# aniketntnu/WordDiffusion

Measured on AMD Instinct MI355X. Metric: denoised 64x256 word images/sec (1000-step DDPM), whole job, higher is better.
Workload: dtype bf16x3; 1 GPU; BASELINE configs[1]: batch 64 per GPU of 64x256 crops = [64,4,8,32] latents, 1000-step DDPM (999 executed steps), base unet.py UNetModel (320 ch, mult (1,1), 4 heads, 339 writers), random-init synthetic weights; variant=base, batch_per_gpu=64, noise_steps=1000, executed_steps_per_image=999, precision=split-bf16 MFMA x3, fp32 accumulate (<=1e-4 of the fp32 reference), output_finite=True

## Files before the change

### worddiffusion_amd/csrc/wd_common.h

```cpp
#pragma once
#include <hip/hip_runtime.h>
#include <stdint.h>

#include "../../include/wdiff_hip.h"

#define WD_CLS_GEMM 0
#define WD_CLS_GNSTATS 1
#define WD_CLS_GNAPPLY 2
#define WD_CLS_LN 3
#define WD_CLS_ATTN 4
#define WD_CLS_OTHER 5
#define WD_CLS_GEMM_OTHER 6
#define WD_CLS_GEMM_REDUCE 7
#define WD_CLS_GEMM_2CU 8
#define WD_CLS_GEMM_WDIRECT 9
#define WD_CLS_FF 10
#define WD_CLS_DW 11
#define WD_CLS_GEMM_Q 12

extern "C" int wd_prof_is_on();
void wd_prof_begin(int cls, hipStream_t s, double flops);
void wd_prof_end(hipStream_t s);

struct WdLaunchScope {
    hipStream_t s;
    bool on;
    WdLaunchScope(int cls, hipStream_t st, double flops = 0.0) : s(st), on(wd_prof_is_on() != 0) {
        if (on) wd_prof_begin(cls, s, flops);
    }
    ~WdLaunchScope() {
        if (on) wd_prof_end(s);
    }
};

static inline int wd_check_launch() {
    hipError_t e = hipGetLastError();
    return e == hipSuccess ? WD_OK : WD_ELAUNCH;
}

__device__ __forceinline__ uint32_t wd_f2bf_bits(float x) {
    uint32_t u = __float_as_uint(x);
    return (u + 0x7FFFu + ((u >> 16) & 1u)) >> 16;
}
__device__ __forceinline__ float wd_bf_bits2f(uint32_t b) { return __uint_as_float(b << 16); }

typedef __attribute__((ext_vector_type(2))) float wd_f32x2;
typedef __attribute__((ext_vector_type(2))) __bf16 wd_bf16x2;
__device__ __forceinline__ uint32_t wd_pack_bf16x2(float a, float b) {
    const wd_f32x2 v = {a, b};
    return __builtin_bit_cast(uint32_t, __builtin_convertvector(v, wd_bf16x2));
}

__device__ __forceinline__ void wd_split1(float x, uint32_t& hi, uint32_t& lo) {
    hi = wd_pack_bf16x2(x, 0.f) & 0xffffu;
    lo = wd_pack_bf16x2(x - __uint_as_float(hi << 16), 0.f) & 0xffffu;
}

__device__ __forceinline__ void wd_split4(const float4 v, uint2& hi, uint2& lo) {
    const uint32_t h01 = wd_pack_bf16x2(v.x, v.y), h23 = wd_pack_bf16x2(v.z, v.w);
    hi = make_uint2(h01, h23);
    lo = make_uint2(wd_pack_bf16x2(v.x - __uint_as_float(h01 << 16), v.y - __uint_as_float(h01 & 0xffff0000u)),
                    wd_pack_bf16x2(v.z - __uint_as_float(h23 << 16), v.w - __uint_as_float(h23 & 0xffff0000u)));
}

__device__ __forceinline__ float wd_silu(float x) { return __fdividef(x, 1.0f + __expf(-x)); }
__device__ __forceinline__ float wd_erf(float x) {
    const float ax = fabsf(x);
    const float t = __fdividef(1.0f, 1.0f + 0.3275911f * ax);
    const float poly = t * (0.254829592f + t * (-0.284496736f + t * (1.421413741f + t * (-1.453152027f + t * 1.061405429f))));
    const float r = 1.0f - poly * __expf(-ax * ax);
    return copysignf(r, x);
}
__device__ __forceinline__ float wd_gelu_erf(float x) { return 0.5f * x * (1.0f + wd_erf(x * 0.70710678118654752440f)); }

template <int CTRL>
__device__ __forceinline__ float wd_dpp(float v) {
    return __int_as_float(__builtin_amdgcn_update_dpp(0, __float_as_int(v), CTRL, 0xf, 0xf, true));
}
__device__ __forceinline__ float wd_row16_sum(float v) {
    v += wd_dpp<0xB1>(v);
    v += wd_dpp<0x4E>(v);
    v += wd_dpp<0x124>(v);
    v += wd_dpp<0x128>(v);
    return v;
}
__device__ __forceinline__ float wd_wave_sum(float v) {
    v += wd_dpp<0xB1>(v);
    v += wd_dpp<0x4E>(v);
    v += wd_dpp<0x124>(v);
    v += wd_dpp<0x128>(v);
    const float r0 = __int_as_float(__builtin_amdgcn_readlane(__float_as_int(v), 0));
    const float r1 = __int_as_float(__builtin_amdgcn_readlane(__float_as_int(v), 16));
    const float r2 = __int_as_float(__builtin_amdgcn_readlane(__float_as_int(v), 32));
    const float r3 = __int_as_float(__builtin_amdgcn_readlane(__float_as_int(v), 48));
    return (r0 + r1) + (r2 + r3);
}
__device__ __forceinline__ float wd_wave_max(float v) {
    v = fmaxf(v, wd_dpp<0xB1>(v));
    v = fmaxf(v, wd_dpp<0x4E>(v));
    v = fmaxf(v, wd_dpp<0x124>(v));
    v = fmaxf(v, wd_dpp<0x128>(v));
    const float r0 = __int_as_float(__builtin_amdgcn_readlane(__float_as_int(v), 0));
    const float r1 = __int_as_float(__builtin_amdgcn_readlane(__float_as_int(v), 16));
    const float r2 = __int_as_float(__builtin_amdgcn_readlane(__float_as_int(v), 32));
    const float r3 = __int_as_float(__builtin_amdgcn_readlane(__float_as_int(v), 48));
    return fmaxf(fmaxf(r0, r1), fmaxf(r2, r3));
}
```

### worddiffusion_amd/csrc/wd_ff.hip

```cpp
#include "wd_gemm_epi.h"

namespace {

constexpr int FNT = 512;
constexpr int FBM = 64;
constexpr int FC = 320;
constexpr int FCH = 128;
constexpr int FRING = 6;
constexpr int F_MAX_INNER = 2048;
constexpr int FGRP = 30;
constexpr uint32_t F_OOB = 0x80000000u;

typedef __attribute__((ext_vector_type(4))) unsigned f_u32x4;

__device__ __forceinline__ int f_lds_off(int row, int ch) { return row * 128 + ((ch ^ ((row >> 1) & 7)) << 4); }

__host__ __device__ __forceinline__ wd_gemm_args ff_epi_args(const wd_ff_args& a, const bool proj, const bool fold) {
    wd_gemm_args e = {};
    e.m = a.m;
    e.n = FC;
    e.hw_out = a.hw_out > 0 ? a.hw_out : 1;
    e.act = WD_ACT_NONE;
    e.out_f32 = a.out_f32;
    e.out_ld = a.out_ld;
    e.out_hi = a.out_hi;
    e.out_lo = a.out_lo;
    e.out_pl_ld = a.out_pl_ld;
    e.ksplit = 1;
    e.stat_part = a.stat_part;
    e.stat_cpg = a.stat_cpg;
    e.bias = !proj ? a.b2 : fold ? a.b32 : a.b3;
    e.resid = proj ? a.resid3 : a.resid;
    e.resid_ld = proj ? a.resid3_ld : a.resid_ld;
    e.dbg = a.dbg;
    return e;
}

__device__ __forceinline__ void ff_epilogue(const wd_gemm_args& e, float* ep, const int m0, const int tid) {
    if ((e.dbg & WD_EPI_BATCH_BIT) && wd_epilogue_batch_ok(e, FBM, FC)) wd_epilogue_rows<FBM, FC, FNT>(e, ep, m0, 0, tid);
    else wd_epilogue_from_image<FBM, FC, FNT>(e, ep, m0, 0, tid);
}

template <int NPASS, bool PROJ, bool FRONT, bool FOLD>
__global__ void __launch_bounds__(FNT, 1) wd_ff_kernel(const wd_ff_args a) {
#if defined(__HIP_DEVICE_COMPILE__)
    static_assert(!FRONT || (NPASS == 3 && PROJ), "the transformer front needs split-bf16 operands and the proj_out tail");
    static_assert(!FOLD || (NPASS == 3 && PROJ), "the folded tail is the proj_out tail in split-bf16");
    constexpr int NPL = (NPASS == 1) ? 1 : 2;
    constexpr int SLAB = 2 * FBM * 128;
    constexpr int A_BYTES = 5 * SLAB;
    constexpr int H_BYTES = 2 * SLAB;
    extern __shared__ __attribute__((aligned(16))) char smem[];
    char* s_a = smem;
    char* s_h = smem + A_BYTES;
    float* s_b1 = reinterpret_cast<float*>(smem + A_BYTES + 2 * H_BYTES);

    const int m0 = blockIdx.x * FBM;
    const int tid = threadIdx.x;
    const int lane = tid & 63;
    const int wave = __builtin_amdgcn_readfirstlane(tid >> 6);
    const int kh = wave >> 2, cg = wave & 3;
    const int l15 = lane & 15, lq = lane >> 4;
    const int nchunk = a.inner / FCH;

    auto make_srd = [](const wd_bf16* p) {
        return __builtin_amdgcn_make_buffer_rsrc(const_cast<wd_bf16*>(p), 0, 0x7FFFFFF0, 0x00020000);
    };
    const __amdgpu_buffer_rsrc_t srd1_hi = make_srd(a.w1_hi), srd1_lo = make_srd(a.w1_lo ? a.w1_lo : a.w1_hi);
    const __amdgpu_buffer_rsrc_t srd2_hi = make_srd(FOLD ? a.w32_hi : a.w2_hi),
                                 srd2_lo = make_srd(FOLD ? a.w32_lo : a.w2_lo ? a.w2_lo : a.w2_hi);
    const __amdgpu_buffer_rsrc_t srd3_hi = make_srd(PROJ ? a.w3_hi : a.w2_hi), srd3_lo = make_srd(PROJ ? (a.w3_lo ? a.w3_lo : a.w3_hi) : a.w2_hi);
    const uint32_t lane16 = lane * 16;
    const int nct1 = (2 * a.inner) >> 4;

    bf16x8 ring[FRING][NPL];
    auto issue = [&](const int slot, const int g, const int j) {
        const bool live = j < nchunk;
        const uint32_t vo = live ? lane16 : F_OOB;
        if (PROJ && !FOLD && g < FRING) {
            const uint32_t so3 = (uint32_t)(((2 * (g / 5) + kh) * (FC / 16) + 5 * cg + g % 5) * 1024);
            const uint32_t so1 = (uint32_t)(((g >> 1) * nct1 + 2 * (j * 8 + wave) + (g & 1)) * 1024);
            const uint32_t so = live ? so1 : so3;
#pragma unroll
            for (int p = 0; p < NPL; ++p) {
                const __amdgpu_buffer_rsrc_t srd = live ? (p ? srd1_lo : srd1_hi) : (p ? srd3_lo : srd3_hi);
                ring[slot][p] = __builtin_bit_cast(bf16x8, __builtin_amdgcn_raw_buffer_load_b128(srd, lane16, so, 0));
            }
        } else if (g < 20) {
            const uint32_t so = (uint32_t)(((g >> 1) * nct1 + 2 * (j * 8 + wave) + (g & 1)) * 1024);
#pragma unroll
            for (int p = 0; p < NPL; ++p)
                ring[slot][p] = __builtin_bit_cast(bf16x8, __builtin_amdgcn_raw_buffer_load_b128(p ? srd1_lo : srd1_hi, vo, live ? so : 0u, 0));
        } else {
            const int q = (g - 20) / 5, t = (g - 20) % 5;
            const uint32_t so = (uint32_t)(((4 * j + 2 * kh + q) * (FC / 16) + 5 * cg + t) * 1024);
#pragma unroll
            for (int p = 0; p < NPL; ++p)
                ring[slot][p] = __builtin_bit_cast(bf16x8, __builtin_amdgcn_raw_buffer_load_b128(p ? srd2_lo : srd2_hi, vo, live ? so : 0u, 0));
        }
    };
    f32x4 acc2[4][5];
    bf16x8 xa[4][NPL];
    auto read_frags = [&](const char* slab_base, const int half) {
        const int ch = half * 4 + lq;
#pragma unroll
        for (int i = 0; i < 4; ++i) {
            const int ao = f_lds_off(i * 16 + l15, ch);
#pragma unroll
            for (int p = 0; p < NPL; ++p) xa[i][p] = *reinterpret_cast<const bf16x8*>(slab_base + p * (FBM * 128) + ao);
        }
    };
    auto mfma12 = [&](f32x4 (&acc)[4], const bf16x8 (&w)[NPL]) {
#pragma unroll
        for (int i = 0; i < 4; ++i) {
            if (NPL == 2) {
                acc[i] = __builtin_amdgcn_mfma_f32_16x16x32_bf16(xa[i][NPL - 1], w[0], acc[i], 0, 0, 0);
                acc[i] = __builtin_amdgcn_mfma_f32_16x16x32_bf16(xa[i][0], w[NPL - 1], acc[i], 0, 0, 0);
            }
            acc[i] = __builtin_amdgcn_mfma_f32_16x16x32_bf16(xa[i][0], w[0], acc[i], 0, 0, 0);
        }
    };
    constexpr int LDE = FC + 4;
    float* ep = reinterpret_cast<float*>(smem);
    auto ksum_to_image = [&]() {
        for (int hh = 0; hh < 2; ++hh) {
            if (kh == hh) {
#pragma unroll
                for (int i = 0; i < 4; ++i)
#pragma unroll
                    for (int t = 0; t < 5; ++t)
#pragma unroll
                        for (int r = 0; r < 4; ++r) {
                            float* pe = ep + (i * 16 + 4 * lq + r) * LDE + cg * 80 + t * 16 + l15;
                            *pe = (hh == 0) ? acc2[i][t][r] : *pe + acc2[i][t][r];
                        }
            }
            __syncthreads();
        }
    };

    auto issue_w3 = [&](const int slot, const int g) {
        const uint32_t so = (uint32_t)(((2 * (g / 5) + kh) * (FC / 16) + 5 * cg + g % 5) * 1024);
#pragma unroll
        for (int p = 0; p < NPL; ++p)
            ring[slot][p] = __builtin_bit_cast(bf16x8, __builtin_amdgcn_raw_buffer_load_b128(p ? srd3_lo : srd3_hi, lane16, so, 0));
    };
    auto fold_product = [&](const int q0, const int q1, const char* slabs) {
        if (q0 == 0) {
#pragma unroll
            for (int i = 0; i < 4; ++i)
#pragma unroll
                for (int t = 0; t < 5; ++t)
#pragma unroll
                    for (int r = 0; r < 4; ++r) acc2[i][t][r] = 0.0f;
        }
#pragma unroll
        for (int g = 0; g < 25; ++g) {
            const int q = g / 5, t = g % 5;
            if (q < q0 || q >= q1) continue;
            if (t == 0) read_frags(slabs + (q - q0) * SLAB, kh);
            {
                f32x4 col[4] = {acc2[0][t], acc2[1][t], acc2[2][t], acc2[3][t]};
                mfma12(col, ring[(g + 5) % FRING]);
#pragma unroll
                for (int i = 0; i < 4; ++i) acc2[i][t] = col[i];
            }
            if (g + FRING < 25) issue_w3((g + 5) % FRING, g + FRING);
            else issue((g + 5) % FRING, g + FRING - 25, 0);
            __builtin_amdgcn_sched_barrier(0);
        }
    };

    if constexpr (FRONT) {
        constexpr int SP = 65, PP = 72, KS32 = FC / 32;
        const int b = m0 / a.hw;
        const int HJ = a.heads * a.L;
        char* fr = s_h + 4096;
        float* s_aff = reinterpret_cast<float*>(fr);
        float* sS = reinterpret_cast<float*>(fr);
        wd_bf16* sP = reinterpret_cast<wd_bf16*>(fr + FBM * SP * 4);
        float* s_vec = reinterpret_cast<float*>(s_h + (FOLD ? 49152 : 40960));
        const float* s_pib = s_vec;
        const float* s_ln2g = s_vec + FC, * s_ln2b = s_vec + 2 * FC, * s_ln3g = s_vec + 3 * FC, * s_ln3b = s_vec + 4 * FC;
        const float* s_xba = s_vec + 5 * FC, * s_xbb = s_vec + 6 * FC;
        const int arow = tid >> 3, ach = tid & 7;
        float4 xv[5][2];
        {
            const float* xrow = a.x_in + (long)(m0 + arow) * a.x_in_ld + ach * 8;
#pragma unroll
            for (int sl = 0; sl < 5; ++sl) {
                xv[sl][0] = *reinterpret_cast<const float4*>(xrow + sl * 64);
                xv[sl][1] = *reinterpret_cast<const float4*>(xrow + sl * 64 + 4);
            }
        }
        const __amdgpu_buffer_rsrc_t srdp_hi = make_srd(a.pi_hi), srdp_lo = make_srd(a.pi_lo);
        auto issue_pi = [&](const int slot, const int g) {
            const uint32_t so = (uint32_t)(((2 * (g / 5) + kh) * (FC / 16) + 5 * cg + g % 5) * 1024);
#pragma unroll
            for (int p = 0; p < NPL; ++p)
                ring[slot][p] = __builtin_bit_cast(bf16x8, __builtin_amdgcn_raw_buffer_load_b128(p ? srdp_lo : srdp_hi, lane16, so, 0));
        };
#pragma unroll
        for (int g = 0; g < FRING; ++g) issue_pi(g, g);
        const int sv = wave < 7 ? wave : 6;
        const float* vsrc = sv == 0 ? a.pi_b : sv == 1 ? a.ln2_gamma : sv == 2 ? a.ln2_beta : sv == 3 ? a.ln3_gamma : sv == 4 ? a.ln3_beta
                            : sv == 5 ? a.xb_a : a.xb_b;
        const float4 vst0 = *reinterpret_cast<const float4*>(vsrc + lane * 4);
        const float4 vst1 = *reinterpret_cast<const float4*>(vsrc + (64 + l15) * 4);
        constexpr int NB1 = 2 * F_MAX_INNER / FNT;
        float b1v[NB1];
        {
            const __amdgpu_buffer_rsrc_t sb1 = __builtin_amdgcn_make_buffer_rsrc(const_cast<float*>(a.b1), 0, a.b1 ? 2 * a.inner * 4 : 0, 0x00020000);
#pragma unroll
            for (int k = 0; k < NB1; ++k)
                b1v[k] = __builtin_bit_cast(float, __builtin_amdgcn_raw_buffer_load_b32(sb1, (uint32_t)(tid + k * FNT) * 4u, 0, 0));
        }
        __builtin_amdgcn_sched_barrier(0);
        for (int e = tid; e < FBM * PP; e += FNT) reinterpret_cast<uint32_t*>(sP)[e] = 0u;
        {
            const int ngp = FC / a.gn_pcpg, ratio = a.gn_cpg / a.gn_pcpg;
            for (int c = tid; c < FC; c += FNT) {
                const int g = c / a.gn_cpg;
                const float gam = a.gn_gamma[c], bet = a.gn_beta[c];
                double su = 0.0, sq = 0.0;
                const int nterm = ratio * a.gn_nchunk;
                int k = 0, ck = 0;
                for (int t0 = 0; t0 < nterm; t0 += 8) {
                    const int k0 = k, ck0 = ck;
                    double2 pv[8];
#pragma unroll
                    for (int u = 0; u < 8; ++u) {
                        const bool live = t0 + u < nterm;
                        const int kk = live ? k : k0, cc = live ? ck : ck0;
                        pv[u] = *reinterpret_cast<const double2*>(a.gn_part + (((long)b * a.gn_nchunk + cc) * ngp + g * ratio + kk) * 2);
                        if (++ck == a.gn_nchunk) {
                            ck = 0;
                            ++k;
                        }
                    }
#pragma unroll
                    for (int u = 0; u < 8; ++u)
                        if (t0 + u < nterm) {
                            su += pv[u].x;
                            sq += pv[u].y;
                        }
                }
                const double n = (double)a.hw * a.gn_cpg;
                const double mu = su / n;
                double var = sq / n - mu * mu;
                if (var < 0.0) var = 0.0;
                const float rstd = (float)(1.0 / sqrt(var + (double)a.gn_eps));
                const float sc = rstd * gam;
                s_aff[2 * c] = sc;
                s_aff[2 * c + 1] = bet - (float)mu * sc;
            }
        }
        __builtin_amdgcn_sched_barrier(0);
        if (wave < 7) {
            *reinterpret_cast<float4*>(s_vec + sv * FC + lane * 4) = vst0;
            *reinterpret_cast<float4*>(s_vec + sv * FC + (64 + l15) * 4) = vst1;
        }
#pragma unroll
        for (int k = 0; k < NB1; ++k)
            if (tid + k * FNT < 2 * a.inner) s_b1[tid + k * FNT] = b1v[k];
        __syncthreads();
#pragma unroll
        for (int sl = 0; sl < 5; ++sl) {
            const float4* tab = reinterpret_cast<const float4*>(s_aff + 2 * (sl * 64 + ach * 8));
            const float4 t0 = tab[0], t1 = tab[1], t2 = tab[2], t3 = tab[3];
            const float4 x0 = xv[sl][0], x1 = xv[sl][1];
            float4 y0, y1;
            y0.x = x0.x * t0.x + t0.y; y0.y = x0.y * t0.z + t0.w; y0.z = x0.z * t1.x + t1.y; y0.w = x0.w * t1.z + t1.w;
            y1.x = x1.x * t2.x + t2.y; y1.y = x1.y * t2.z + t2.w; y1.z = x1.z * t3.x + t3.y; y1.w = x1.w * t3.z + t3.w;
            uint2 h0, l0, h1, l1;
// ... 183 lines not shown
                        for (int t = 0; t < 5; ++t) o[ri][t] = __builtin_amdgcn_mfma_f32_16x16x32_bf16(al, mh[ks][t], o[ri][t], 0, 0, 0);
#pragma unroll
                        for (int t = 0; t < 5; ++t) o[ri][t] = __builtin_amdgcn_mfma_f32_16x16x32_bf16(ah, ml[ks][t], o[ri][t], 0, 0, 0);
#pragma unroll
                        for (int t = 0; t < 5; ++t) o[ri][t] = __builtin_amdgcn_mfma_f32_16x16x32_bf16(ah, mh[ks][t], o[ri][t], 0, 0, 0);
                    }
#pragma unroll
                for (int ri = 0; ri < 2; ++ri)
#pragma unroll
                    for (int t = 0; t < 5; ++t)
#pragma unroll
                        for (int r = 0; r < 4; ++r) ep[((2 * rp + ri) * 16 + 4 * lq + r) * LDE + (5 * cg + t) * 16 + l15] = o[ri][t][r];
            }
            if (ps == 0) {
                issue_mq(a.mq_b);
            } else {
#pragma unroll
                for (int g = 0; g < FRING; ++g) {
                    if (FOLD) issue_w3((g + 5) % FRING, g);
                    else issue(g, g, 0);
                }
                __builtin_amdgcn_sched_barrier(0);
            }
            __syncthreads();
#pragma unroll
            for (int pp = 0; pp < 2; ++pp)
#pragma unroll
                for (int i = 0; i < 5; ++i) {
                    const int n = (l15 + 16 * i) * 4, row = wave * 8 + pp * 4 + lq;
                    const float4 bi = *reinterpret_cast<const float4*>(xb + n);
                    const float4 at = *reinterpret_cast<const float4*>(ep + row * LDE + n);
                    const float4 x = xr[pp][i];
                    xr[pp][i] = make_float4(at.x + bi.x + x.x, at.y + bi.y + x.y, at.z + bi.z + x.z, at.w + bi.w + x.w);
                }
            __syncthreads();
        }
        if constexpr (!FOLD) {
#pragma unroll
            for (int pp = 0; pp < 2; ++pp)
#pragma unroll
                for (int i = 0; i < 5; ++i)
                    *reinterpret_cast<float4*>(a.tok2 + (long)(m0 + wave * 8 + pp * 4 + lq) * FC + (l15 + 16 * i) * 4) = xr[pp][i];
        } else {
            const __amdgpu_buffer_rsrc_t st2 = __builtin_amdgcn_make_buffer_rsrc(a.tok2, 0, a.tok2 ? 0x7FFFFFF0 : 0, 0x00020000);
            float4* park = reinterpret_cast<float4*>(s_a);
            auto planes = [&](const int pp, const int i, const int i0) {
                const int n = (l15 + 16 * i) * 4, row = wave * 8 + pp * 4 + lq;
                uint2 hi, lo;
                wd_split4(xr[pp][i], hi, lo);
                char* d = s_h + (i - i0) * SLAB + f_lds_off(row, (n & 63) >> 3) + (n & 7) * 2;
                *reinterpret_cast<uint2*>(d) = hi;
                *reinterpret_cast<uint2*>(d + FBM * 128) = lo;
            };
#pragma unroll
            for (int pp = 0; pp < 2; ++pp)
#pragma unroll
                for (int i = 0; i < 5; ++i) {
                    const int n = (l15 + 16 * i) * 4, row = wave * 8 + pp * 4 + lq;
                    __builtin_amdgcn_raw_buffer_store_b128(__builtin_bit_cast(f_u32x4, xr[pp][i]), st2, (uint32_t)(((m0 + row) * FC + n) * 4), 0, 0);
                    park[(pp * 5 + i) * FNT + tid] = xr[pp][i];
                    if (i < 3) planes(pp, i, 0);
                }
            __syncthreads();
            fold_product(0, 3, s_h);
            __syncthreads();
#pragma unroll
            for (int pp = 0; pp < 2; ++pp)
#pragma unroll
                for (int i = 3; i < 5; ++i) {
                    xr[pp][i] = park[(pp * 5 + i) * FNT + tid];
                    planes(pp, i, 3);
                }
            __syncthreads();
            fold_product(3, 5, s_h);
#pragma unroll
            for (int pp = 0; pp < 2; ++pp)
#pragma unroll
                for (int i = 0; i < 5; ++i) xr[pp][i] = park[(pp * 5 + i) * FNT + tid];
            __syncthreads();
        }
        ln_rows(s_ln3g, s_ln3b);
    } else {
#pragma unroll
    for (int g = 0; g < FRING; ++g) {
        if (FOLD) issue_w3((g + 5) % FRING, g);
        else issue(g, g, 0);
    }
    if constexpr (FOLD) {
        const int arow = tid >> 3, ach = tid & 7;
        const bool rok = m0 + arow < a.m;
        const float* xrow = a.resid + (long)(rok ? m0 + arow : 0) * a.resid_ld + ach * 8;
        float4 xv[5][2];
#pragma unroll
        for (int sl = 0; sl < 5; ++sl) {
            xv[sl][0] = *reinterpret_cast<const float4*>(xrow + sl * 64);
            xv[sl][1] = *reinterpret_cast<const float4*>(xrow + sl * 64 + 4);
        }
#pragma unroll
        for (int sl = 0; sl < 5; ++sl) {
            const float4 z = make_float4(0.f, 0.f, 0.f, 0.f);
            uint2 h0, l0, h1, l1;
            wd_split4(rok ? xv[sl][0] : z, h0, l0);
            wd_split4(rok ? xv[sl][1] : z, h1, l1);
            char* dst = s_a + sl * SLAB + f_lds_off(arow, ach);
            *reinterpret_cast<f_u32x4*>(dst) = f_u32x4{h0.x, h0.y, h1.x, h1.y};
            *reinterpret_cast<f_u32x4*>(dst + FBM * 128) = f_u32x4{l0.x, l0.y, l1.x, l1.y};
        }
        __syncthreads();
        fold_product(0, 5, s_a);
        __syncthreads();
    }

    {
        const __amdgpu_buffer_rsrc_t sx_hi = make_srd(a.x_hi), sx_lo = make_srd(a.x_lo ? a.x_lo : a.x_hi);
        const int arow = tid >> 3, ach = tid & 7;
        const uint32_t vo = (m0 + arow < a.m) ? (uint32_t)(m0 + arow) * (uint32_t)(a.x_ld * 2) + (uint32_t)(ach * 16) : F_OOB;
        f_u32x4 v[5][NPL];
#pragma unroll
        for (int sl = 0; sl < 5; ++sl)
#pragma unroll
            for (int p = 0; p < NPL; ++p) v[sl][p] = __builtin_amdgcn_raw_buffer_load_b128(p ? sx_lo : sx_hi, vo, sl * 128, 0);
        const int dst = f_lds_off(arow, ach);
#pragma unroll
        for (int sl = 0; sl < 5; ++sl)
#pragma unroll
            for (int p = 0; p < NPL; ++p) *reinterpret_cast<f_u32x4*>(s_a + sl * SLAB + p * (FBM * 128) + dst) = v[sl][p];
        for (int i = tid; i < 2 * a.inner; i += FNT) s_b1[i] = a.b1 ? a.b1[i] : 0.0f;
    }
    }
    __syncthreads();

    if constexpr (!FOLD) {
#pragma unroll
        for (int i = 0; i < 4; ++i)
#pragma unroll
            for (int t = 0; t < 5; ++t)
#pragma unroll
                for (int r = 0; r < 4; ++r) acc2[i][t][r] = 0.0f;
    }

    for (int j = 0; j < nchunk; ++j) {
        char* hbuf = s_h + (j & 1) * H_BYTES;
        f32x4 ax[4], ag[4];
#pragma unroll
        for (int i = 0; i < 4; ++i)
#pragma unroll
            for (int r = 0; r < 4; ++r) {
                ax[i][r] = 0.0f;
                ag[i][r] = 0.0f;
            }
#pragma unroll
        for (int g = 0; g < 20; ++g) {
            if ((g & 1) == 0) read_frags(s_a + (g >> 2) * SLAB, (g >> 1) & 1);
            if (g & 1) mfma12(ag, ring[g % FRING]);
            else mfma12(ax, ring[g % FRING]);
            if (g + FRING < FGRP) issue(g % FRING, g + FRING, j);
            else issue(g % FRING, g + FRING - FGRP, j + 1);
            __builtin_amdgcn_sched_barrier(0);
        }
        {
            const int hcol = (j * 8 + wave) * 32 + l15;
            const float bx = s_b1[hcol], bg = s_b1[hcol + 16];
            const int slab = wave >> 2, ch = (wave & 3) * 2 + (l15 >> 3), e = (l15 & 7) * 2;
#pragma unroll
            for (int i = 0; i < 4; ++i)
#pragma unroll
                for (int r = 0; r < 4; ++r) {
                    const float h = (ax[i][r] + bx) * wd_gelu_erf(ag[i][r] + bg);
                    uint32_t hb, lb;
                    wd_split1(h, hb, lb);
                    char* p = hbuf + slab * SLAB + f_lds_off(i * 16 + lq * 4 + r, ch) + e;
                    *reinterpret_cast<unsigned short*>(p) = (unsigned short)hb;
                    if (NPL == 2) *reinterpret_cast<unsigned short*>(p + FBM * 128) = (unsigned short)lb;
                }
        }
        __syncthreads();
#pragma unroll
        for (int g = 20; g < FGRP; ++g) {
            const int q = (g - 20) / 5, t = (g - 20) % 5;
            if (t == 0) read_frags(hbuf + kh * SLAB, q);
            {
                f32x4 col[4] = {acc2[0][t], acc2[1][t], acc2[2][t], acc2[3][t]};
                mfma12(col, ring[g % FRING]);
#pragma unroll
                for (int i = 0; i < 4; ++i) acc2[i][t] = col[i];
            }
            if (g + FRING < FGRP) issue(g % FRING, g + FRING, j);
            else issue(g % FRING, g + FRING - FGRP, j + 1);
            __builtin_amdgcn_sched_barrier(0);
        }
    }

    __syncthreads();
    ksum_to_image();
    const wd_gemm_args e = ff_epi_args(a, PROJ, FOLD);
    if constexpr (!PROJ) {
        ff_epilogue(e, ep, m0, tid);
    } else if constexpr (FOLD) {
        ff_epilogue(e, ep, m0, tid);
    } else {
        constexpr int ROWB = LDE * 4;
        const float* resid = FRONT ? a.tok2 : a.resid;
        const int resid_ld = FRONT ? FC : a.resid_ld;
        if (FRONT) asm volatile("s_waitcnt vmcnt(0)" ::: "memory");
        {
            float4 v[10];
#pragma unroll
            for (int it = 0; it < 10; ++it) {
                const int idx = it * 64 + lane, row = wave * 8 + idx / 80, c = (idx % 80) * 4;
                const int m = m0 + row;
                float4 x = *reinterpret_cast<const float4*>(ep + row * LDE + c);
                if (a.b2) {
                    const float4 q = *reinterpret_cast<const float4*>(a.b2 + c);
                    x.x += q.x; x.y += q.y; x.z += q.z; x.w += q.w;
                }
                if (resid && m < a.m) {
                    const float4 q = *reinterpret_cast<const float4*>(resid + (long)m * resid_ld + c);
                    x.x += q.x; x.y += q.y; x.z += q.z; x.w += q.w;
                }
                v[it] = x;
            }
            asm volatile("s_waitcnt lgkmcnt(0)" ::: "memory");
            __builtin_amdgcn_sched_barrier(0);
#pragma unroll
            for (int it = 0; it < 10; ++it) {
                const int idx = it * 64 + lane, row = wave * 8 + idx / 80, c = (idx % 80) * 4;
                uint2 hh, ll;
                wd_split4(v[it], hh, ll);
                char* rowp = reinterpret_cast<char*>(ep) + row * ROWB;
                *reinterpret_cast<uint2*>(rowp + c * 2) = hh;
                if (NPL == 2) *reinterpret_cast<uint2*>(rowp + 640 + c * 2) = ll;
            }
        }
        __syncthreads();
#pragma unroll
        for (int i = 0; i < 4; ++i)
#pragma unroll
            for (int t = 0; t < 5; ++t)
#pragma unroll
                for (int r = 0; r < 4; ++r) acc2[i][t][r] = 0.0f;
#pragma unroll
        for (int g = 0; g < 25; ++g) {
            const int q = g / 5, t = g % 5;
            if (t == 0) {
                const int ks = 2 * q + kh;
#pragma unroll
                for (int i = 0; i < 4; ++i) {
                    const char* rp = reinterpret_cast<const char*>(ep) + (i * 16 + l15) * ROWB + (ks * 4 + lq) * 16;
#pragma unroll
                    for (int p = 0; p < NPL; ++p) xa[i][p] = *reinterpret_cast<const bf16x8*>(rp + p * 640);
                }
            }
            {
                f32x4 col[4] = {acc2[0][t], acc2[1][t], acc2[2][t], acc2[3][t]};
                mfma12(col, ring[g % FRING]);
#pragma unroll
                for (int i = 0; i < 4; ++i) acc2[i][t] = col[i];
            }
            if (g + FRING < 25) {
                const int g2 = g + FRING;
                const uint32_t so3 = (uint32_t)(((2 * (g2 / 5) + kh) * (FC / 16) + 5 * cg + g2 % 5) * 1024);
#pragma unroll
                for (int p = 0; p < NPL; ++p)
                    ring[g % FRING][p] = __builtin_bit_cast(bf16x8, __builtin_amdgcn_raw_buffer_load_b128(p ? srd3_lo : srd3_hi, lane16, so3, 0));
            }
            __builtin_amdgcn_sched_barrier(0);
        }
        __syncthreads();
        ksum_to_image();
        ff_epilogue(e, ep, m0, tid);
    }
#endif
}

template <int NPASS, bool PROJ, bool FRONT = false, bool FOLD = false>
int launch_ff(const wd_ff_args& a, hipStream_t st) {
    constexpr int max_smem = 5 * 2 * FBM * 128 + 2 * 2 * 2 * FBM * 128 + 2 * F_MAX_INNER * 4;
    constexpr int red_smem = FBM * (FC + 4) * 4 + WD_STAT_SCRATCH;
    static_assert(max_smem <= 160 * 1024 && red_smem <= max_smem, "LDS budget");
    const int loop_smem = max_smem - 2 * (F_MAX_INNER - a.inner) * 4;
    const int smem = loop_smem > red_smem ? loop_smem : red_smem;
    static bool attr_done = false;
    if (!attr_done) {
        if (hipFuncSetAttribute(reinterpret_cast<const void*>(&wd_ff_kernel<NPASS, PROJ, FRONT, FOLD>), hipFuncAttributeMaxDynamicSharedMemorySize,
                                max_smem) != hipSuccess)
            return WD_ELAUNCH;
        attr_done = true;
    }
    const int nb = (a.m + FBM - 1) / FBM;
    const double fl = 2.0 * (double)a.m * (3.0 * (double)a.inner * FC + (PROJ ? (double)FC * FC : 0.0) +
                                           (FRONT ? (double)FC * FC + 4.0 * a.heads * a.L * FC : 0.0));
    WdLaunchScope scope(WD_CLS_FF, st, fl);
    hipLaunchKernelGGL((wd_ff_kernel<NPASS, PROJ, FRONT, FOLD>), dim3(nb), dim3(FNT), smem, st, a);
    return wd_check_launch();
}

}

extern "C" int wd_ff_args_bytes(void) { return (int)sizeof(wd_ff_args); }

extern "C" int wd_ff_supported(int c, int inner) { return (c == FC && inner > 0 && inner % FCH == 0 && inner <= F_MAX_INNER) ? 1 : 0; }

static int wd_ff_resolve(const wd_ff_args& in, wd_ff_args& a) {
    a = in;
    if (!wd_ff_supported(a.c, a.inner) || a.m <= 0 || (a.npass != 1 && a.npass != 3)) return WD_EINVAL;
    const bool front = a.x_in != nullptr;
    if (!a.w1_hi || !a.w2_hi || (a.npass == 3 && (!a.w1_lo || !a.w2_lo))) return WD_EINVAL;
    if (!front && (!a.x_hi || (a.npass == 3 && !a.x_lo) || a.x_ld % 8 || a.x_ld < a.c)) return WD_EINVAL;
    if (!a.out_f32 && !a.out_hi) return WD_EINVAL;
    if ((a.out_ld | a.resid_ld | a.out_pl_ld) & 3) return WD_EINVAL;
    if (a.resid && a.resid_ld <= 0) return WD_EINVAL;
    if ((long)a.m * a.x_ld * 2 >= 0x7FFFFFF0L || (long)2 * a.inner * a.c * 2 >= 0x7FFFFFF0L) return WD_EINVAL;
    const bool proj = a.w3_hi != nullptr;
    const bool fold = a.w32_hi != nullptr;
    if (fold && (!proj || a.npass != 3 || !a.w32_lo || !a.b32 || (!front && !a.resid) || (long)a.m * FC * 4 >= 0x7FFFFFF0L))
        return WD_EINVAL;
    if (proj && ((a.npass == 3 && !a.w3_lo) || (a.resid3 && (a.resid3_ld <= 0 || (a.resid3_ld & 3))))) return WD_EINVAL;
    if (a.stat_part && (a.stat_cpg <= 0 || FC % a.stat_cpg || a.hw_out <= 0 || !(a.hw_out % FBM == 0 || FBM % a.hw_out == 0) ||
                        (FBM > a.hw_out && FBM / a.hw_out > WD_STAT_MAXNS)))
        return WD_EINVAL;
    if (front) {
        if (a.npass != 3 || !proj || a.x_in_ld < a.c || a.x_in_ld % 4 || a.hw <= 0 || a.hw % FBM || a.m % a.hw) return WD_EINVAL;
        if (!a.gn_part || a.gn_nchunk <= 0 || a.gn_pcpg <= 0 || a.gn_cpg <= 0 || a.gn_cpg % a.gn_pcpg || FC % a.gn_cpg ||
            !a.gn_gamma || !a.gn_beta)
            return WD_EINVAL;
        if (!a.pi_hi || !a.pi_lo || !a.pi_b || !a.ln2_gamma || !a.ln2_beta || !a.ln3_gamma || !a.ln3_beta || (!a.tok2 && !fold)) return WD_EINVAL;
        if (!a.mq_a || !a.mot_a || !a.xb_a || !a.mq_b || !a.mot_b || !a.xb_b || !wd_xattn_supported(a.c, a.heads, a.L)) return WD_EINVAL;
// ... 28 lines not shown
```

### worddiffusion_amd/csrc/wd_gemm_epi.h

```cpp
#pragma once
#include "wd_common.h"
#include "wd_gemm_priv.h"

typedef __attribute__((ext_vector_type(8))) __bf16 bf16x8;
typedef __attribute__((ext_vector_type(16))) float f32x16;
typedef __attribute__((ext_vector_type(4))) float f32x4;

namespace {

constexpr int WD_STAT_SCRATCH = 40 * 1024;
constexpr int WD_STAT_MAXNS = 2;

__host__ __device__ __forceinline__ bool wd_epilogue_vec_ok(const wd_gemm_args& a) {
    return (((a.out_ld | a.rowvec_ld | a.resid_ld | a.out_pl_ld) & 3) == 0) &&
           (((reinterpret_cast<uintptr_t>(a.bias) | reinterpret_cast<uintptr_t>(a.rowvec) |
              reinterpret_cast<uintptr_t>(a.resid) | reinterpret_cast<uintptr_t>(a.out_f32)) & 15) == 0) &&
           (((reinterpret_cast<uintptr_t>(a.out_hi) | reinterpret_cast<uintptr_t>(a.out_lo)) & 7) == 0);
}

constexpr int WD_EPI_BATCH_MAX_LD = 1 << 22;
__host__ __device__ __forceinline__ bool wd_epilogue_batch_shape(const wd_gemm_args& a, const int bm, const int bn) {
    const bool pitches = (!a.out_f32 || a.out_ld < WD_EPI_BATCH_MAX_LD) && (!a.out_hi || a.out_pl_ld < WD_EPI_BATCH_MAX_LD) &&
                         (!a.resid || a.resid_ld < WD_EPI_BATCH_MAX_LD);
    return a.ksplit <= 1 && (a.act == WD_ACT_NONE || a.act == WD_ACT_SILU) && !a.ln_gamma && !a.gn_gamma && !a.a32 && !a.resid_rows &&
// ... 22 lines not shown
    const float p[4] = {t.p.x, t.p.y, t.p.z, t.p.w}, s[4] = {t.s.x, t.s.y, t.s.z, t.s.w}, q[4] = {t.q.x, t.q.y, t.q.z, t.q.w};
    const double n = (double)t.n;
#pragma unroll
    for (int j = 0; j < 4; ++j) {
        const double pj = (double)p[j], sj = (double)s[j];
        su[j] = n * pj + sj;
        sq[j] = n * pj * pj + 2.0 * pj * sj + (double)q[j];
    }
}

template <int NT>
__device__ __forceinline__ void wd_stat_reduce(double* scr, const int ns, const int nrl, const int ngt, const int bn, const int cpg,
                                               const int tid) {
    for (int it = tid; it < ns * ngt * nrl; it += NT) {
        const int l = it % nrl, g = (it / nrl) % ngt, sidx2 = it / (nrl * ngt);
        double* p = scr + (long)(sidx2 * nrl + l) * bn + g * cpg;
        double su = 0.0;
        for (int cc = 0; cc < cpg; ++cc) su += p[cc];
        __builtin_amdgcn_s_waitcnt(0xC07F);
        p[0] = su;
    }
}

template <int BM, int BN, int NT>
__device__ __forceinline__ void wd_stat_handover(const wd_gemm_args& a, float* ep, const int m0, const int n0, const int tid,
                                                 const WdStatAcc& st, const int cur_s, const float* park, const int nrl, const int rl,
                                                 const int c, const int rps) {
    constexpr int LDE = BN + 4;
    const int ns = BM > a.hw_out ? BM / a.hw_out : 1;
    double ssum[4] = {0.0, 0.0, 0.0, 0.0}, ssq[4] = {0.0, 0.0, 0.0, 0.0};
    double s0[4] = {0.0, 0.0, 0.0, 0.0}, q0[4] = {0.0, 0.0, 0.0, 0.0};
    if (cur_s == 0 && ns > 1) {
        wd_stat_finish(st, s0, q0);
    } else {
        wd_stat_finish(st, ssum, ssq);
        if (cur_s != 0) {
            WdStatAcc pv;
            pv.p = *reinterpret_cast<const float4*>(park);
            pv.s = *reinterpret_cast<const float4*>(park + 4);
            pv.q = *reinterpret_cast<const float4*>(park + 2 * nrl * BN);
            pv.n = __float_as_int(park[2 * nrl * BN + 4]);
            wd_stat_finish(pv, s0, q0);
        }
    }
    const int cpg = a.stat_cpg;
    const int ngt = BN / cpg;
    const int nchunk = a.hw_out > BM ? a.hw_out / BM : 1;
    const int ngs = a.n / cpg;
    double* scr = reinterpret_cast<double*>(ep + BM * LDE);
    const int nq = 2 * ns * nrl * BN * (int)sizeof(double) <= WD_STAT_SCRATCH ? 2 : 1;
    for (int q0i = 0; q0i < 2; q0i += nq) {
        if (q0i) __syncthreads();
        if (rl < nrl && c < BN) {
            for (int qq = 0; qq < nq; ++qq) {
                const bool sq = q0i + qq;
                const double* lo = ns > 1 ? (sq ? q0 : s0) : (sq ? ssq : ssum);
                double* o = scr + ((long)(qq * ns) * nrl + rl) * BN + c;
                *reinterpret_cast<double2*>(o) = make_double2(lo[0], lo[1]);
                *reinterpret_cast<double2*>(o + 2) = make_double2(lo[2], lo[3]);
                if (ns > 1) {
                    const double* hi = sq ? ssq : ssum;
                    o += nrl * BN;
                    *reinterpret_cast<double2*>(o) = make_double2(hi[0], hi[1]);
                    *reinterpret_cast<double2*>(o + 2) = make_double2(hi[2], hi[3]);
                }
            }
        }
        __syncthreads();
        wd_stat_reduce<NT>(scr, nq * ns, nrl, ngt, BN, cpg, tid);
        __syncthreads();
        for (int it = tid; it < nq * ns * ngt; it += NT) {
            const int g = it % ngt, qs = it / ngt, sidx2 = qs % ns, qq = qs / ns;
            const int mrow = m0 + sidx2 * rps;
            if (mrow >= a.m || n0 + g * cpg >= a.n) continue;
            double su = 0.0;
            for (int l = 0; l < nrl; ++l) su += scr[(long)(qs * nrl + l) * BN + g * cpg];
            const int b = mrow / a.hw_out;
            const int chunk = (mrow - b * a.hw_out) / BM;
            a.stat_part[(((long)b * nchunk + chunk) * ngs + n0 / cpg + g) * 2 + q0i + qq] = su;
        }
    }
}

template <int BM, int BN, int NT, bool WS = false>
__device__ __forceinline__ void wd_epilogue_from_image(const wd_gemm_args& a, float* ep, const int m0, const int n0,
                                                       const int tid, const int nslab = 1) {
    constexpr int LDE = BN + 4;
    const bool geglu = a.act == WD_ACT_GEGLU;
    const int ocols = geglu ? BN / 2 : BN;
    const int oc4 = ocols / 4;
    const int nout = geglu ? a.n / 2 : a.n;
    const int no0 = geglu ? n0 / 2 : n0;
    const bool stats = a.stat_part != nullptr;
    const bool vec = wd_epilogue_vec_ok(a);
    if (!vec) {
        for (int i = tid; i < BM * ocols; i += NT) {
            const int row = i / ocols, c = i - row * ocols;
            const int m = m0 + row, no = no0 + c;
            if (m >= a.m || no >= nout) continue;
            float v;
            if (geglu) {
                const float x = ep[row * LDE + c] + (a.bias ? a.bias[n0 + c] : 0.f);
                const float g = ep[row * LDE + c + BN / 2] + (a.bias ? a.bias[n0 + c + BN / 2] : 0.f);
                v = x * wd_gelu_erf(g);
            } else {
                v = ep[row * LDE + c] + (a.bias ? a.bias[no] : 0.f);
            }
            if (a.rowvec) v += a.rowvec[(long)(m / a.hw_out) * a.rowvec_ld + no];
            if (a.resid) v += a.resid[(a.resid_rows ? (long)a.resid_rows[m] : (long)m) * a.resid_ld + no];
            if (a.act == WD_ACT_SILU) v = wd_silu(v);
            if (stats || a.ln_gamma) ep[row * LDE + c] = v;
            if (a.out_f32) a.out_f32[(long)m * a.out_ld + no] = v;
            if (a.out_hi && !a.ln_gamma) {
                uint32_t hb, lb;
                wd_split1(v, hb, lb);
                a.out_hi[(long)m * a.out_pl_ld + no] = (wd_bf16)hb;
                if (a.out_lo) a.out_lo[(long)m * a.out_pl_ld + no] = (wd_bf16)lb;
            }
        }
    } else {
        const int nrl = NT / oc4;
        const int rl = tid / oc4, c = (tid - rl * oc4) * 4;
        const int no = no0 + c;
        const int rps = BM > a.hw_out ? a.hw_out : BM;
        const int rps_sh = 31 - __clz(rps);
        const int hw_sh = (a.hw_out & (a.hw_out - 1)) == 0 ? 31 - __clz(a.hw_out) : -1;
        WdStatAcc st;
        wd_stat_reset(st);
        float* park = ep + BM * LDE + 2 * ((long)rl * BN + c);
        int cur_s = 0;
        if (rl < nrl && no < nout) {
            float4 bx = make_float4(0, 0, 0, 0), bg = bx;
            if (a.bias) {
                bx = *reinterpret_cast<const float4*>(a.bias + (geglu ? n0 + c : no));
                if (geglu) bg = *reinterpret_cast<const float4*>(a.bias + n0 + c + BN / 2);
            }
            for (int row = rl; row < BM; row += nrl) {
                const int m = m0 + row;
                if (m >= a.m) break;
                float4 v;
                if constexpr (WS) {
                    const float* p = a.ws + (long)m * a.n + n0 + c;
                    const long total = (long)a.m * a.n;
                    v = *reinterpret_cast<const float4*>(p);
                    for (int sp = 1; sp < nslab; ++sp) {
                        const float4 q = *reinterpret_cast<const float4*>(p + (long)sp * total);
                        v.x += q.x; v.y += q.y; v.z += q.z; v.w += q.w;
                    }
                } else {
                    v = *reinterpret_cast<const float4*>(ep + row * LDE + c);
                }
                if (geglu) {
                    const float4 g = *reinterpret_cast<const float4*>(ep + row * LDE + c + BN / 2);
                    v.x = (v.x + bx.x) * wd_gelu_erf(g.x + bg.x);
                    v.y = (v.y + bx.y) * wd_gelu_erf(g.y + bg.y);
                    v.z = (v.z + bx.z) * wd_gelu_erf(g.z + bg.z);
                    v.w = (v.w + bx.w) * wd_gelu_erf(g.w + bg.w);
                } else {
                    v.x += bx.x; v.y += bx.y; v.z += bx.z; v.w += bx.w;
                }
                if (a.rowvec) {
                    const int bi = hw_sh >= 0 ? m >> hw_sh : m / a.hw_out;
                    const float4 q = *reinterpret_cast<const float4*>(a.rowvec + (long)bi * a.rowvec_ld + no);
                    v.x += q.x; v.y += q.y; v.z += q.z; v.w += q.w;
                }
                if (a.resid) {
                    const long rr = a.resid_rows ? (long)a.resid_rows[m] : (long)m;
                    const float4 q = *reinterpret_cast<const float4*>(a.resid + rr * a.resid_ld + no);
                    v.x += q.x; v.y += q.y; v.z += q.z; v.w += q.w;
                }
                if (a.act == WD_ACT_SILU) {
                    v.x = wd_silu(v.x); v.y = wd_silu(v.y); v.z = wd_silu(v.z); v.w = wd_silu(v.w);
                }
                if (stats) {
                    const int sidx2 = row >> rps_sh;
                    if (sidx2 != cur_s) {
                        *reinterpret_cast<float4*>(park) = st.p;
                        *reinterpret_cast<float4*>(park + 4) = st.s;
                        *reinterpret_cast<float4*>(park + 2 * nrl * BN) = st.q;
                        park[2 * nrl * BN + 4] = __int_as_float(st.n);
                        wd_stat_reset(st);
                        cur_s = sidx2;
                    }
                    wd_stat_add(st, v);
                }
                if (a.ln_gamma) {
                    if constexpr (!WS) *reinterpret_cast<float4*>(ep + row * LDE + c) = v;
                }
                if (no + 3 < nout) {
                    if (a.out_f32) *reinterpret_cast<float4*>(a.out_f32 + (long)m * a.out_ld + no) = v;
                    if (a.out_hi && !a.ln_gamma) {
                        uint2 hh, ll;
                        wd_split4(v, hh, ll);
                        *reinterpret_cast<uint2*>(a.out_hi + (long)m * a.out_pl_ld + no) = hh;
                        if (a.out_lo) *reinterpret_cast<uint2*>(a.out_lo + (long)m * a.out_pl_ld + no) = ll;
                    }
                } else {
                    const float e[4] = {v.x, v.y, v.z, v.w};
                    for (int j = 0; j < 4 && no + j < nout; ++j) {
                        if (a.out_f32) a.out_f32[(long)m * a.out_ld + no + j] = e[j];
                        if (a.out_hi) {
                            uint32_t hb, lb;
                            wd_split1(e[j], hb, lb);
                            a.out_hi[(long)m * a.out_pl_ld + no + j] = (wd_bf16)hb;
                            if (a.out_lo) a.out_lo[(long)m * a.out_pl_ld + no + j] = (wd_bf16)lb;
                        }
                    }
                }
            }
        }
        if (stats) wd_stat_handover<BM, BN, NT>(a, ep, m0, n0, tid, st, cur_s, park, nrl, rl, c, rps);
    }
    if (a.ln_gamma) {
        __syncthreads();
        constexpr int NW = NT / 64;
        const int lane = tid & 63, wv = tid >> 6;
        const bool has0 = lane * 4 < BN, has1 = (64 + lane) * 4 < BN;
        float4 gq[2], bq[2];
#pragma unroll
        for (int h = 0; h < 2; ++h) {
            gq[h] = bq[h] = make_float4(0.f, 0.f, 0.f, 0.f);
            if (h ? has1 : has0) {
                gq[h] = *reinterpret_cast<const float4*>(a.ln_gamma + (h * 64 + lane) * 4);
                bq[h] = *reinterpret_cast<const float4*>(a.ln_beta + (h * 64 + lane) * 4);
            }
        }
        for (int row = wv; row < BM; row += NW) {
            const int m = m0 + row;
            if (m >= a.m) break;
            const float* rp = ep + row * LDE;
            float4 x0 = make_float4(0.f, 0.f, 0.f, 0.f), x1 = x0;
            if (has0) x0 = *reinterpret_cast<const float4*>(rp + lane * 4);
            if (has1) x1 = *reinterpret_cast<const float4*>(rp + (64 + lane) * 4);
            const float mean = wd_wave_sum((x0.x + x0.y) + (x0.z + x0.w) + (x1.x + x1.y) + (x1.z + x1.w)) * (1.0f / BN);
            float d = 0.f;
            if (has0) d += (x0.x - mean) * (x0.x - mean) + (x0.y - mean) * (x0.y - mean) + (x0.z - mean) * (x0.z - mean) + (x0.w - mean) * (x0.w - mean);
            if (has1) d += (x1.x - mean) * (x1.x - mean) + (x1.y - mean) * (x1.y - mean) + (x1.z - mean) * (x1.z - mean) + (x1.w - mean) * (x1.w - mean);
            const float rstd = rsqrtf(wd_wave_sum(d) * (1.0f / BN) + a.ln_eps);
#pragma unroll
            for (int h = 0; h < 2; ++h) {
                if (!(h ? has1 : has0)) continue;
                const int c = (h * 64 + lane) * 4;
                const float4 x = h ? x1 : x0;
                const float4 g = gq[h], b = bq[h];
                float4 y;
                y.x = (x.x - mean) * rstd * g.x + b.x; y.y = (x.y - mean) * rstd * g.y + b.y;
                y.z = (x.z - mean) * rstd * g.z + b.z; y.w = (x.w - mean) * rstd * g.w + b.w;
                uint2 hh, ll;
                wd_split4(y, hh, ll);
                *reinterpret_cast<uint2*>(a.out_hi + (long)m * a.out_pl_ld + c) = hh;
                if (a.out_lo) *reinterpret_cast<uint2*>(a.out_lo + (long)m * a.out_pl_ld + c) = ll;
            }
        }
    }
}

typedef __attribute__((ext_vector_type(4))) unsigned wd_u32x4;
typedef __attribute__((ext_vector_type(2))) unsigned wd_u32x2;
constexpr uint32_t WD_EPI_OOB = 0x80000000u;

template <int BM, int BN, int NT>
__device__ __forceinline__ void wd_epilogue_rows(const wd_gemm_args& a, float* ep, const int m0, const int n0, const int tid) {
    constexpr int LDE = BN + 4, Q = BN / 4, NRL = NT / Q, KEEP = (BM + NRL - 1) / NRL;
    const int rl = tid / Q, c = (tid - rl * Q) * 4;
    const bool live = rl < NRL;
    const bool planes = a.out_hi != nullptr;
    auto window = [&](const void* p, const long row0, const int ld, const int rows, const int esz) {
        const char* base = reinterpret_cast<const char*>(p) + (row0 * ld + n0) * esz;
        return __builtin_amdgcn_make_buffer_rsrc(const_cast<char*>(base), 0, p ? ((rows - 1) * ld + BN) * esz : 0, 0x00020000);
    };
    const __amdgpu_buffer_rsrc_t s_bias = window(a.bias, 0, 0, 1, 4);
    const __amdgpu_buffer_rsrc_t s_rv = window(a.rowvec, a.rowvec ? m0 / a.hw_out : 0, a.rowvec_ld, 1, 4);
    const __amdgpu_buffer_rsrc_t s_res = window(a.resid, m0, a.resid_ld, BM, 4);
    const __amdgpu_buffer_rsrc_t s_f32 = window(a.out_f32, m0, a.out_ld, BM, 4);
    const __amdgpu_buffer_rsrc_t s_hi = window(a.out_hi, m0, a.out_pl_ld, BM, 2);
    const __amdgpu_buffer_rsrc_t s_lo = window(planes ? a.out_lo : nullptr, m0, a.out_pl_ld, BM, 2);
    auto as_f4 = [](const wd_u32x4 u) { return __builtin_bit_cast(float4, u); };

    float4 v[KEEP], r[KEEP];
#pragma unroll
    for (int k = 0; k < KEEP; ++k) {
        const int row = rl + k * NRL;
        v[k] = *reinterpret_cast<const float4*>(ep + (row < BM ? row : BM - 1) * LDE + c);
    }
    const uint32_t vo_c = live ? (uint32_t)c * 4u : WD_EPI_OOB;
    const float4 bx = as_f4(__builtin_amdgcn_raw_buffer_load_b128(s_bias, vo_c, 0, 0));
    const float4 rv = as_f4(__builtin_amdgcn_raw_buffer_load_b128(s_rv, vo_c, 0, 0));
#pragma unroll
    for (int k = 0; k < KEEP; ++k) {
        const int row = rl + k * NRL;
        const uint32_t vo = (live && row < BM) ? ((uint32_t)row * (uint32_t)a.resid_ld + (uint32_t)c) * 4u : WD_EPI_OOB;
        r[k] = as_f4(__builtin_amdgcn_raw_buffer_load_b128(s_res, vo, 0, 0));
    }
    __builtin_amdgcn_s_waitcnt(0x0070);
    __builtin_amdgcn_sched_barrier(0);
    const bool has_rv = a.rowvec != nullptr, has_res = a.resid != nullptr, silu = a.act == WD_ACT_SILU, stats = a.stat_part != nullptr;
    WdStatAcc st;
    wd_stat_reset(st);
#pragma unroll
    for (int k = 0; k < KEEP; ++k) {
        const int row = rl + k * NRL;
        const bool ok = live && row < BM;
        float4 x = v[k];
        x.x += bx.x; x.y += bx.y; x.z += bx.z; x.w += bx.w;
        if (has_rv) {
            x.x += rv.x; x.y += rv.y; x.z += rv.z; x.w += rv.w;
        }
        if (has_res) {
            x.x += r[k].x; x.y += r[k].y; x.z += r[k].z; x.w += r[k].w;
        }
// ... 190 lines not shown
```

Measured before the change: 37.19 images/s.

## Transpose FF GEMM1 MFMA operands and vectorize GEGLU epilogue with packed math

The fused feed-forward kernel now issues its first GEMM with the weight and activation operands swapped, so each lane holds four consecutive hidden columns instead of four rows. The GEGLU epilogue can then load bias as float4, evaluate GELU on packed float2 vectors, split to bf16 hi/lo four values at a time, and write 8-byte LDS stores instead of scattered 2-byte stores. SiLU and erf also switch from fast division to the hardware reciprocal builtin. The change targets epilogue ALU and LDS store cost on the FF path. The risk is that the transposed layout must still match what the second GEMM reads, and the reciprocal instruction carries slightly different rounding.

```diff
diff --git a/worddiffusion_amd/csrc/wd_common.h b/worddiffusion_amd/csrc/wd_common.h
--- a/worddiffusion_amd/csrc/wd_common.h
+++ b/worddiffusion_amd/csrc/wd_common.h
@@ -63,15 +63,28 @@
                     wd_pack_bf16x2(v.z - __uint_as_float(h23 << 16), v.w - __uint_as_float(h23 & 0xffff0000u)));
 }
 
-__device__ __forceinline__ float wd_silu(float x) { return __fdividef(x, 1.0f + __expf(-x)); }
+__device__ __forceinline__ float wd_rcp(float x) { return __builtin_amdgcn_rcpf(x); }
+
+__device__ __forceinline__ float wd_silu(float x) { return x * wd_rcp(1.0f + __expf(-x)); }
 __device__ __forceinline__ float wd_erf(float x) {
     const float ax = fabsf(x);
-    const float t = __fdividef(1.0f, 1.0f + 0.3275911f * ax);
+    const float t = wd_rcp(1.0f + 0.3275911f * ax);
     const float poly = t * (0.254829592f + t * (-0.284496736f + t * (1.421413741f + t * (-1.453152027f + t * 1.061405429f))));
     const float r = 1.0f - poly * __expf(-ax * ax);
     return copysignf(r, x);
 }
 __device__ __forceinline__ float wd_gelu_erf(float x) { return 0.5f * x * (1.0f + wd_erf(x * 0.70710678118654752440f)); }
+__device__ __forceinline__ wd_f32x2 wd_erf2(wd_f32x2 x) {
+    const wd_f32x2 ax = {fabsf(x.x), fabsf(x.y)};
+    const wd_f32x2 d = 1.0f + 0.3275911f * ax;
+    const wd_f32x2 t = {wd_rcp(d.x), wd_rcp(d.y)};
+    const wd_f32x2 poly = t * (0.254829592f + t * (-0.284496736f + t * (1.421413741f + t * (-1.453152027f + t * 1.061405429f))));
+    const wd_f32x2 s = -ax * ax;
+    const wd_f32x2 ex = {__expf(s.x), __expf(s.y)};
+    const wd_f32x2 r = 1.0f - poly * ex;
+    return wd_f32x2{copysignf(r.x, x.x), copysignf(r.y, x.y)};
+}
+__device__ __forceinline__ wd_f32x2 wd_gelu_erf2(wd_f32x2 x) { return 0.5f * x * (1.0f + wd_erf2(x * 0.70710678118654752440f)); }
 
 template <int CTRL>
 __device__ __forceinline__ float wd_dpp(float v) {
diff --git a/worddiffusion_amd/csrc/wd_ff.hip b/worddiffusion_amd/csrc/wd_ff.hip
--- a/worddiffusion_amd/csrc/wd_ff.hip
+++ b/worddiffusion_amd/csrc/wd_ff.hip
@@ -120,6 +120,16 @@
             acc[i] = __builtin_amdgcn_mfma_f32_16x16x32_bf16(xa[i][0], w[0], acc[i], 0, 0, 0);
         }
     };
+    auto mfma12_t = [&](f32x4 (&acc)[4], const bf16x8 (&w)[NPL]) {
+#pragma unroll
+        for (int i = 0; i < 4; ++i) {
+            if (NPL == 2) {
+                acc[i] = __builtin_amdgcn_mfma_f32_16x16x32_bf16(w[0], xa[i][NPL - 1], acc[i], 0, 0, 0);
+                acc[i] = __builtin_amdgcn_mfma_f32_16x16x32_bf16(w[NPL - 1], xa[i][0], acc[i], 0, 0, 0);
+            }
+            acc[i] = __builtin_amdgcn_mfma_f32_16x16x32_bf16(w[0], xa[i][0], acc[i], 0, 0, 0);
+        }
+    };
     constexpr int LDE = FC + 4;
     float* ep = reinterpret_cast<float*>(smem);
     auto ksum_to_image = [&]() {
@@ -609,27 +619,28 @@
 #pragma unroll
         for (int g = 0; g < 20; ++g) {
             if ((g & 1) == 0) read_frags(s_a + (g >> 2) * SLAB, (g >> 1) & 1);
-            if (g & 1) mfma12(ag, ring[g % FRING]);
-            else mfma12(ax, ring[g % FRING]);
+            if (g & 1) mfma12_t(ag, ring[g % FRING]);
+            else mfma12_t(ax, ring[g % FRING]);
             if (g + FRING < FGRP) issue(g % FRING, g + FRING, j);
             else issue(g % FRING, g + FRING - FGRP, j + 1);
             __builtin_amdgcn_sched_barrier(0);
         }
         {
-            const int hcol = (j * 8 + wave) * 32 + l15;
-            const float bx = s_b1[hcol], bg = s_b1[hcol + 16];
-            const int slab = wave >> 2, ch = (wave & 3) * 2 + (l15 >> 3), e = (l15 & 7) * 2;
-#pragma unroll
-            for (int i = 0; i < 4; ++i)
-#pragma unroll
-                for (int r = 0; r < 4; ++r) {
-                    const float h = (ax[i][r] + bx) * wd_gelu_erf(ag[i][r] + bg);
-                    uint32_t hb, lb;
-                    wd_split1(h, hb, lb);
-                    char* p = hbuf + slab * SLAB + f_lds_off(i * 16 + lq * 4 + r, ch) + e;
-                    *reinterpret_cast<unsigned short*>(p) = (unsigned short)hb;
-                    if (NPL == 2) *reinterpret_cast<unsigned short*>(p + FBM * 128) = (unsigned short)lb;
-                }
+            const float* pb = s_b1 + (j * 8 + wave) * 32 + 4 * lq;
+            const float4 bx = *reinterpret_cast<const float4*>(pb), bg = *reinterpret_cast<const float4*>(pb + 16);
+            const wd_f32x2 bx01 = {bx.x, bx.y}, bx23 = {bx.z, bx.w}, bg01 = {bg.x, bg.y}, bg23 = {bg.z, bg.w};
+            char* hq = hbuf + (wave >> 2) * SLAB + (lq & 1) * 8;
+            const int ch = (wave & 3) * 2 + (lq >> 1);
+#pragma unroll
+            for (int i = 0; i < 4; ++i) {
+                const wd_f32x2 h01 = (wd_f32x2{ax[i][0], ax[i][1]} + bx01) * wd_gelu_erf2(wd_f32x2{ag[i][0], ag[i][1]} + bg01);
+                const wd_f32x2 h23 = (wd_f32x2{ax[i][2], ax[i][3]} + bx23) * wd_gelu_erf2(wd_f32x2{ag[i][2], ag[i][3]} + bg23);
+                uint2 hb, lb;
+                wd_split4(make_float4(h01.x, h01.y, h23.x, h23.y), hb, lb);
+                char* p = hq + f_lds_off(i * 16 + l15, ch);
+                *reinterpret_cast<uint2*>(p) = hb;
+                if (NPL == 2) *reinterpret_cast<uint2*>(p + FBM * 128) = lb;
+            }
         }
         __syncthreads();
 #pragma unroll
diff --git a/worddiffusion_amd/csrc/wd_gemm_epi.h b/worddiffusion_amd/csrc/wd_gemm_epi.h
--- a/worddiffusion_amd/csrc/wd_gemm_epi.h
+++ b/worddiffusion_amd/csrc/wd_gemm_epi.h
@@ -198,10 +198,9 @@
                 }
                 if (geglu) {
                     const float4 g = *reinterpret_cast<const float4*>(ep + row * LDE + c + BN / 2);
-                    v.x = (v.x + bx.x) * wd_gelu_erf(g.x + bg.x);
-                    v.y = (v.y + bx.y) * wd_gelu_erf(g.y + bg.y);
-                    v.z = (v.z + bx.z) * wd_gelu_erf(g.z + bg.z);
-                    v.w = (v.w + bx.w) * wd_gelu_erf(g.w + bg.w);
+                    const wd_f32x2 h01 = (wd_f32x2{v.x, v.y} + wd_f32x2{bx.x, bx.y}) * wd_gelu_erf2(wd_f32x2{g.x, g.y} + wd_f32x2{bg.x, bg.y});
+                    const wd_f32x2 h23 = (wd_f32x2{v.z, v.w} + wd_f32x2{bx.z, bx.w}) * wd_gelu_erf2(wd_f32x2{g.z, g.w} + wd_f32x2{bg.z, bg.w});
+                    v = make_float4(h01.x, h01.y, h23.x, h23.y);
                 } else {
                     v.x += bx.x; v.y += bx.y; v.z += bx.z; v.w += bx.w;
                 }
```

After: 37.77 images/s (median of 6 runs). 1.02x the previous value.
